# groupeLIAMG/ttcr

Measured on AMD Instinct MI355X. Metric: Mnodes/s per sweep-iteration (512^3 fp32 grid, first-order FSM), higher is better.
Workload: dtype f32

## Files before the change

ttcr_amd/csrc/fsm_capi.hip:

```cpp
#include <hip/hip_runtime.h>

#include <algorithm>
#include <atomic>
#include <chrono>
#include <condition_variable>
#include <cmath>
#include <cstdio>
#include <cstdlib>
#include <cstring>
#include <limits>
#include <map>
#include <memory>
#include <mutex>
#include <sstream>
#include <stdexcept>
#include <string>
#include <thread>
#include <vector>

#include "../../include/ttcr_amd.h"
#include "fsm_kernels.h"
#include "fsm_fast_api.h"
#include "fsm_tape_api.h"
#include "fsm_adjoint_api.h"
// ... 492 lines not shown
                    const int ja = std::max(j0 - 2 * H, 0), jb = std::min(jm + 2 * H, geom.NJ - 1);
                    const int ka = std::max(k0 - 2 * H, 0), kb = std::min(km + 2 * H, geom.NK - 1);
                    const int ja2 = rj != prj ? geom.NJ - 1 - jb : ja, jb2 = rj != prj ? geom.NJ - 1 - ja : jb;
                    const int ka2 = rk != prk ? geom.NK - 1 - kb : ka, kb2 = rk != prk ? geom.NK - 1 - ka : kb;
                    for (int tk = ka2 / PK; tk <= kb2 / PK; ++tk)
                        for (int tj = ja2 / PJ; tj <= jb2 / PJ; ++tj) t = std::max(t, tf[(size_t)(d - 1) * n_patches + (size_t)tk * npj + tj]);
                }
                ts[me] = t;
                tf[me] = t + ((jm - j0) + (km - k0) + geom.NF + C - 1) / C + 1.0;
            }
        }
        std::vector<uint32_t> idx((size_t)n_patches * ndir);
        size_t q = 0;
        std::vector<uint32_t> ent((size_t)n_patches * ndir);
        std::vector<double> key((size_t)n_patches * ndir);
        for (int d = 0; d < ndir; ++d)
            for (uint32_t e : diag_order) {
                const int TJ = e & 0xffffu, TK = e >> 16;
                ent[q] = (uint32_t)TJ | ((uint32_t)TK << 14) | ((uint32_t)d << 28);
                key[q] = ts[(size_t)d * n_patches + (size_t)TK * npj + TJ];
                idx[q] = (uint32_t)q;
                ++q;
            }
        std::stable_sort(idx.begin(), idx.end(), [&](uint32_t a2, uint32_t b2) { return key[a2] < key[b2]; });
        for (uint32_t i2 : idx) out.push_back(ent[i2]);
        return out;
    }

    template <int DIM, int H>
    void launch_sweeps_persistent(int batch) {
        constexpr int C0 = ChunkCfg<T, DIM>::C;
        if constexpr (DIM == 3 && C0 == 8) {
            const int below = H == 2 ? weno_c16_below : sizeof(T) == 4 ? std::numeric_limits<int>::max() : f64_c16_below;
            if (NS == 1 && mode == 2 && (lone_chunk == 16 || fast_now<H>()) && batch < below) {
                launch_sweeps_persistent_ns<DIM, H, 1, 16, true>(batch);
                return;
            }
        }
        if (H == 2 && DIM == 3 && NS == 2 && batch >= weno_ch4_min && C0 == 8) {
            if (NS == 2) launch_sweeps_persistent_ns<DIM, H, 2, (H == 2 && DIM == 3) ? 4 : C0>(batch);
            else launch_sweeps_persistent_ns<DIM, H, 1, (H == 2 && DIM == 3) ? 4 : C0>(batch);
        } else {
            if (NS == 2) launch_sweeps_persistent_ns<DIM, H, 2, C0>(batch); else launch_sweeps_persistent_ns<DIM, H, 1, C0>(batch);
        }
    }

    template <int DIM, int H, int NSV, int CH, bool XS_ONLY = false>
    void launch_sweeps_persistent_ns(int batch) {
        using C = TileCfg<T, DIM>;
        PersistArgs<T> pa;
        SweepArgs<T>& a = pa.s;
        constexpr bool NO_PRE = CH == 16 && H == 1 && DIM == 3;
        const size_t dyn_lds = NO_PRE ? 0 : xs_dyn_lds(batch);
        a.tt = d_tt.p;
        a.ts = NS;
        a.lmask = d_lmask.p;
        a.frozen = d_mask.p;
        a.bbox = d_bbox.p;
        a.change = d_change.p;
        a.slots = d_slots.p;
        a.tiles = nullptr;
        a.g = geom;
        a.prof = d_prof.p;
        a.mask_words = (uint32_t)mask_words;
        a.dx = dx;
        a.dz = dz;
        a.w = 0;
        a.variant = DIM == 3 ? 0 : (dx == dz ? 1 : 2);
        pa.order = d_order.p;
        pa.sync = d_sync.p;
        pa.n_patches = n_patches;
        pa.batch = batch;
        pa.timeout_ticks = 300000000ull;
        pa.stamp = d_stamp.p;
        pa.iter_ptr = d_iter.p;
        pa.evals = d_evals.p;
        pa.nbf = nbf; pa.nbj = nbj; pa.nbk = nbk;
        pa.ndir = DIM == 3 ? 8 : 4;
        pa.skip = skip_now(batch) ? (std::getenv("TTCR_FSM_SKIP_ALL_DIRTY") ? 2 : 1) : 0;
        pa.cmap = d_cmap.p;
        pa.cw = cmap_words;
        pa.sw = std::getenv("TTCR_FSM_NO_SW") ? nullptr : d_sw.p;
        pa.n_sw_groups = n_groups();
        pa.n_sw_sweeps = sw_sweeps;

        const size_t wg_cap = (fsm_looped(DIM == 3, H) && persist_wgs > 0) ? (size_t)persist_wgs : ~(size_t)0;
        const dim3 block(C::PJ * C::PK), grid((unsigned)std::min<size_t>((size_t)n_patches * batch, wg_cap));
        const int ndir = DIM == 3 ? 8 : 4;
        {
            const bool pre_ = mode == 2 && !NO_PRE && (DIM == 2 || batch >= pre_min || dyn_lds > 0);
            char nm[160];
            std::snprintf(nm, sizeof nm, "fsm_sweep_persistent<%s,%d,%d,%d,%s,%s,%d,%d,%s,%s>", sizeof(T) == 4 ? "float" : "double", C::PJ, C::PK, CH,
                          DIM == 3 ? "true" : "false", skip_now(batch) ? "true" : "false", H, NSV, mode == 2 ? "true" : "false", pre_ ? "true" : "false");
            last_kernel = nm;
        }
        if (mode == 2) {
            pa.ssh = d_ssh.p;
            pa.ssh_stride = ssh_stride;
            pa.dir = 0;
            a.rf = a.rj = a.rk = a.rev = 0;
            a.s_sheared = nullptr;
            pa.timeout_ticks = 1000000000ull;
            const dim3 gridx((unsigned)std::min<size_t>((size_t)n_patches * batch * ndir, wg_cap));
            pa.order = d_order_xs[H == 2 ? 1 : 0][batch < time_order_below ? 1 : 0].p;
            const bool pre = DIM == 2 || batch >= pre_min || dyn_lds > 0;
            if constexpr (std::is_same<T, float>::value) {
                if (fast_now<H>() && (H == 1 || NSV == 1)) {
                    const FastCfg fc{H, DIM, NSV, CH, skip_now(batch), NO_PRE ? false : pre};
                    last_kernel.insert(last_kernel.size() - 1, ",1");
                    const hipError_t e = fsm_fast_launch(pa, fc, gridx.x, dyn_lds, stream);
                    if (e == hipErrorInvalidValue) throw std::logic_error("arith = 1: no such kernel (" + last_kernel + ")");
                    HIP_CHECK(e);
                    return;
                }
            }
            if constexpr (NO_PRE) {
                (void)pre;
                if (skip_now(batch))
                    fsm_sweep_persistent<T, C::PJ, C::PK, CH, DIM == 3, true, H, NSV, true><<<gridx, block, dyn_lds, stream>>>(pa);
                else
                    fsm_sweep_persistent<T, C::PJ, C::PK, CH, DIM == 3, false, H, NSV, true><<<gridx, block, dyn_lds, stream>>>(pa);
            } else {
                if (skip_now(batch) && pre)
                    fsm_sweep_persistent<T, C::PJ, C::PK, CH, DIM == 3, true, H, NSV, true, true><<<gridx, block, dyn_lds, stream>>>(pa);
                else if (skip_now(batch))
                    fsm_sweep_persistent<T, C::PJ, C::PK, CH, DIM == 3, true, H, NSV, true><<<gridx, block, dyn_lds, stream>>>(pa);
                else if (pre)
                    fsm_sweep_persistent<T, C::PJ, C::PK, CH, DIM == 3, false, H, NSV, true, true><<<gridx, block, dyn_lds, stream>>>(pa);
                else
                    fsm_sweep_persistent<T, C::PJ, C::PK, CH, DIM == 3, false, H, NSV, true><<<gridx, block, dyn_lds, stream>>>(pa);
            }
            HIP_CHECK(hipGetLastError());
            return;
        }
        if (fast_now<H>() && H == 1) throw ValueError("option 'arith' = 1 needs whole-iteration launches (option 'mode' = 2)");
        if constexpr (XS_ONLY) throw std::logic_error("launch_sweeps_persistent_ns: whole-iteration launches only");
        else {
        pa.ssh = nullptr;
        pa.ssh_stride = 0;
        static const int RX2[4] = {0, 1, 1, 0}, RZ2[4] = {0, 0, 1, 1};
        for (int d = 0; d < ndir; ++d) {
            int fam;
            if (DIM == 3) {
                a.rf = d & 1; a.rj = (d >> 1) & 1; a.rk = (d >> 2) & 1;
                a.rev = a.rk;
                fam = (a.rf ^ a.rk) | ((a.rj ^ a.rk) << 1);
            } else {
                a.rj = RX2[d]; a.rf = RZ2[d]; a.rk = 0;
                a.rev = a.rj;
                fam = a.rf ^ a.rj;
            }
            a.s_sheared = d_ssh.p + (size_t)fam * ssh_stride;
            pa.dir = d;
            if (skip_now(batch))
                fsm_sweep_persistent<T, C::PJ, C::PK, CH, DIM == 3, true, H, NSV, false><<<grid, block, 0, stream>>>(pa);
            else
                fsm_sweep_persistent<T, C::PJ, C::PK, CH, DIM == 3, false, H, NSV, false><<<grid, block, 0, stream>>>(pa);
        }
        HIP_CHECK(hipGetLastError());
        }
    }

    void build_tile_lists(int PJ, int PK, int BL) {
        std::vector<uint32_t> all;
        tile_off.assign(n_launch, 0);
        tile_cnt.assign(n_launch, 0);
        for (int w = 0; w < n_launch; ++w) {
            tile_off[w] = (int)all.size();
            for (int m = 0; m <= geom.npj + geom.npk - 2; ++m) {
                const int L0 = BL * w - m * (BL - 1);
                for (int TK = std::max(0, m - geom.npj + 1); TK <= std::min(m, geom.npk - 1); ++TK) {
                    const int TJ = m - TK;
                    const int j0 = TJ * PJ, k0 = TK * PK;
                    const int jmaxp = std::min(j0 + PJ, geom.NJ) - 1, kmaxp = std::min(k0 + PK, geom.NK) - 1;
// ... 3350 lines not shown
```

ttcr_amd/csrc/fsm_fast.hip:

```cpp
#include "fsm_fast_api.h"

namespace ttcr_amd {

template <int PJ, int PK, int C, bool IS3D, bool SKIP, int NS, bool PRE, int H = 1>
static hipError_t launch_one(const PersistArgs<float>& pa, unsigned wgs, size_t dyn_lds, hipStream_t stream) {
    fsm_sweep_persistent<float, PJ, PK, C, IS3D, SKIP, H, NS, true, PRE, 1><<<dim3(wgs), dim3(PJ * PK), dyn_lds, stream>>>(pa);
    return hipGetLastError();
}

hipError_t fsm_fast_launch(const PersistArgs<float>& pa, const FastCfg& c, unsigned wgs, size_t dyn_lds, hipStream_t stream) {
    if (c.h == 2) {
#ifndef FSM_FAST_MIN
        if (c.ns != 1) return hipErrorInvalidValue;
        if (c.dim == 3 && c.chunk == 16) {
            if (c.skip) return c.pre ? launch_one<16, 16, 16, true, true, 1, true, 2>(pa, wgs, dyn_lds, stream)
                                     : launch_one<16, 16, 16, true, true, 1, false, 2>(pa, wgs, dyn_lds, stream);
            return c.pre ? launch_one<16, 16, 16, true, false, 1, true, 2>(pa, wgs, dyn_lds, stream)
                         : launch_one<16, 16, 16, true, false, 1, false, 2>(pa, wgs, dyn_lds, stream);
        }
        if (c.dim == 3 && c.chunk == 8) {
            if (c.skip) return c.pre ? launch_one<16, 16, 8, true, true, 1, true, 2>(pa, wgs, dyn_lds, stream)
                                     : launch_one<16, 16, 8, true, true, 1, false, 2>(pa, wgs, dyn_lds, stream);
            return c.pre ? launch_one<16, 16, 8, true, false, 1, true, 2>(pa, wgs, dyn_lds, stream)
                         : launch_one<16, 16, 8, true, false, 1, false, 2>(pa, wgs, dyn_lds, stream);
        }
        if (c.dim == 2 && c.chunk == 16 && c.pre)
            return c.skip ? launch_one<64, 1, 16, false, true, 1, true, 2>(pa, wgs, dyn_lds, stream)
                          : launch_one<64, 1, 16, false, false, 1, true, 2>(pa, wgs, dyn_lds, stream);
#endif
        return hipErrorInvalidValue;
    }
    if (c.dim == 3 && c.ns == 1 && c.chunk == 16 && !c.pre)
        return c.skip ? launch_one<16, 16, 16, true, true, 1, false>(pa, wgs, dyn_lds, stream)
                      : launch_one<16, 16, 16, true, false, 1, false>(pa, wgs, dyn_lds, stream);
#ifndef FSM_FAST_MIN
    if (c.dim == 3 && c.ns == 2 && c.chunk == 8) {
        if (c.skip) return c.pre ? launch_one<16, 16, 8, true, true, 2, true>(pa, wgs, dyn_lds, stream)
                                 : launch_one<16, 16, 8, true, true, 2, false>(pa, wgs, dyn_lds, stream);
        return c.pre ? launch_one<16, 16, 8, true, false, 2, true>(pa, wgs, dyn_lds, stream)
                     : launch_one<16, 16, 8, true, false, 2, false>(pa, wgs, dyn_lds, stream);
    }
    if (c.dim == 2 && c.ns == 1 && c.chunk == 16 && c.pre)
        return c.skip ? launch_one<64, 1, 16, false, true, 1, true>(pa, wgs, dyn_lds, stream)
                      : launch_one<64, 1, 16, false, false, 1, true>(pa, wgs, dyn_lds, stream);
#endif
    return hipErrorInvalidValue;
}

}
```

ttcr_amd/csrc/fsm_fast_api.h:

```cpp
#pragma once
#include "fsm_kernels.h"

namespace ttcr_amd {

struct FastCfg {
    int h;
    int dim;
    int ns;
    int chunk;
    bool skip;
    bool pre;
};
hipError_t fsm_fast_launch(const PersistArgs<float>& pa, const FastCfg& c, unsigned wgs, size_t dyn_lds, hipStream_t stream);

}
```

ttcr_amd/csrc/fsm_kernels.h:

```cpp
#pragma once
#include <hip/hip_runtime.h>
#include <stdint.h>
#include <type_traits>

namespace ttcr_amd {

constexpr int FSM_BRICK = 16;

template <typename T> struct real_traits;
template <> struct real_traits<float> {
    static __host__ __device__ constexpr float max() { return 3.402823466e+38f; }
    static __device__ __forceinline__ float inf() { return __builtin_huge_valf(); }
};
template <> struct real_traits<double> {
    static __host__ __device__ constexpr double max() { return 1.7976931348623157e+308; }
    static __device__ __forceinline__ double inf() { return __builtin_huge_val(); }
};

__device__ __forceinline__ uint32_t idx_u32(double v) { return v < 0 ? 0u : (v >= 4294967295.0 ? 4294967295u : (uint32_t)v); }

__device__ __forceinline__ float rmin(float a, float b) { return a < b ? a : b; }
__device__ __forceinline__ double rmin(double a, double b) { return a < b ? a : b; }
__device__ __forceinline__ float rmax(float a, float b) { return a < b ? b : a; }
__device__ __forceinline__ double rmax(double a, double b) { return a < b ? b : a; }
// ... 691 lines not shown
__device__ __forceinline__ float lane_above(float x, float edge) {
    return __uint_as_float((unsigned)__builtin_amdgcn_update_dpp((int)__float_as_uint(edge), (int)__float_as_uint(x), 0x130, 0xf, 0xf, false));
}
__device__ __forceinline__ double lane_below(double x, double edge) {
    const unsigned long long u = (unsigned long long)__double_as_longlong(x), e = (unsigned long long)__double_as_longlong(edge);
    const unsigned lo = (unsigned)__builtin_amdgcn_update_dpp((int)(unsigned)e, (int)(unsigned)u, 0x138, 0xf, 0xf, false);
    const unsigned hi = (unsigned)__builtin_amdgcn_update_dpp((int)(unsigned)(e >> 32), (int)(unsigned)(u >> 32), 0x138, 0xf, 0xf, false);
    return __longlong_as_double((long long)(((unsigned long long)hi << 32) | lo));
}
__device__ __forceinline__ double lane_above(double x, double edge) {
    const unsigned long long u = (unsigned long long)__double_as_longlong(x), e = (unsigned long long)__double_as_longlong(edge);
    const unsigned lo = (unsigned)__builtin_amdgcn_update_dpp((int)(unsigned)e, (int)(unsigned)u, 0x130, 0xf, 0xf, false);
    const unsigned hi = (unsigned)__builtin_amdgcn_update_dpp((int)(unsigned)(e >> 32), (int)(unsigned)(u >> 32), 0x130, 0xf, 0xf, false);
    return __longlong_as_double((long long)(((unsigned long long)hi << 32) | lo));
}

template <typename T, int NS> struct Pack;
template <typename T> struct Pack<T, 1> { T v[1]; };
template <typename T> struct alignas(2 * sizeof(T)) Pack<T, 2> { T v[2]; };

template <typename T, int NS>
__device__ __forceinline__ Pack<T, NS> pack_fill(T x) {
    Pack<T, NS> p;
#pragma unroll
    for (int l = 0; l < NS; ++l) p.v[l] = x;
    return p;
}
__device__ __forceinline__ Pack<float, 1> ld_sc1(const Pack<float, 1>* p) { Pack<float, 1> r; r.v[0] = ld_sc1(&p->v[0]); return r; }
__device__ __forceinline__ Pack<double, 1> ld_sc1(const Pack<double, 1>* p) { Pack<double, 1> r; r.v[0] = ld_sc1(&p->v[0]); return r; }
__device__ __forceinline__ Pack<float, 2> ld_sc1(const Pack<float, 2>* p) {
    const unsigned long long u = __hip_atomic_load((const unsigned long long*)p, __ATOMIC_RELAXED, __HIP_MEMORY_SCOPE_AGENT);
    Pack<float, 2> r;
    r.v[0] = __uint_as_float((unsigned)u);
    r.v[1] = __uint_as_float((unsigned)(u >> 32));
    return r;
}
__device__ __forceinline__ Pack<double, 2> ld_sc1(const Pack<double, 2>* p) {
    Pack<double, 2> r;
    r.v[0] = ld_sc1(&p->v[0]);
    r.v[1] = ld_sc1(&p->v[1]);
    return r;
}
__device__ __forceinline__ void st_sc1(Pack<float, 1>* p, Pack<float, 1> x) { st_sc1(&p->v[0], x.v[0]); }
__device__ __forceinline__ void st_sc1(Pack<double, 1>* p, Pack<double, 1> x) { st_sc1(&p->v[0], x.v[0]); }
__device__ __forceinline__ void st_sc1(Pack<float, 2>* p, Pack<float, 2> x) {
    const unsigned long long u = (unsigned long long)__float_as_uint(x.v[0]) | ((unsigned long long)__float_as_uint(x.v[1]) << 32);
    __hip_atomic_store((unsigned long long*)p, u, __ATOMIC_RELAXED, __HIP_MEMORY_SCOPE_AGENT);
}
__device__ __forceinline__ void st_sc1(Pack<double, 2>* p, Pack<double, 2> x) {
    st_sc1(&p->v[0], x.v[0]);
    st_sc1(&p->v[1], x.v[1]);
}

__host__ __device__ constexpr bool fsm_looped(bool is3d, int h) { return is3d && h == 1; }

__device__ __forceinline__ int kmaxp_of(int k0, int NK, int PK) { return (k0 + PK < NK ? k0 + PK : NK) - 1; }
template <typename T, int PJ, int PK, int C, bool IS3D, bool SKIP, int H, int NS, bool XS, bool PRE, int AR = 0>
__device__ __forceinline__ bool fsm_sweep_unit(const PersistArgs<T>& pa) {
    static_assert(AR == 0 || std::is_same<T, float>::value, "tolerance-grade arithmetic: fp32 kernels");
    constexpr bool LOOPED = fsm_looped(IS3D, H);
    using P = Pack<T, NS>;
    constexpr int NT = PJ * PK;
    constexpr int RJ = PJ + 2 * H;
    constexpr int NROWS = IS3D ? RJ * (PK + 2 * H) : RJ;
    constexpr int NQ = C + 2 * H;
    constexpr int RS = NQ | 1;
    constexpr int NUP = IS3D ? H * (PJ + PK) : H;
    constexpr int NDH = IS3D ? H * (PJ + PK) : H;
    constexpr int RPI = NT / C;
    constexpr int NOWN = C;
    constexpr int NHI = (NDH + RPI - 1) / RPI;
    constexpr int NUPI = (NUP + RPI - 1) / RPI;
    static_assert(NT % C == 0 && (IS3D || PK == 1) && C <= FSM_BRICK && (H == 1 || H == 2), "tile shape");
    static_assert(C - 1 <= FSM_XPAD, "the rows of a chunk are read from the sheared copies without a wrap");
    static_assert(!(SKIP && FSM_EARLY_PUB > 0), "FSM_EARLY_PUB is a tuning option of the kernels without exact skipping");
    const SweepArgs<T>& a = pa.s;
    const unsigned epoch = (unsigned)pa.iter_ptr[1] + (XS ? 0u : (unsigned)pa.dir);
    const int e2 = (int)(epoch % 3u) + 1;
    auto dec_prog = [&](int raw_) -> int { return (int)((unsigned)raw_ >> 30) == e2 ? (raw_ & 0x3fffffff) : 0; };
    auto ld_raw = [&](const int* p_) -> int { return __hip_atomic_load(p_, __ATOMIC_RELAXED, __HIP_MEMORY_SCOPE_AGENT); };
    auto ld_prog = [&](const int* p_) -> int { return dec_prog(ld_raw(p_)); };
    auto st_prog = [&](int* p_, int v_) {
        __hip_atomic_store(p_, (int)(((unsigned)e2 << 30) | (unsigned)v_), __ATOMIC_RELAXED, __HIP_MEMORY_SCOPE_AGENT);
    };
    auto ld_cmap = [&](const unsigned long long* p_) -> unsigned {
        const unsigned long long v_ = __hip_atomic_load(p_, __ATOMIC_RELAXED, __HIP_MEMORY_SCOPE_AGENT);
        return (unsigned)(v_ >> 32) == epoch ? (unsigned)v_ : 0u;
    };
    auto st_cmap = [&](unsigned long long* p_, unsigned v_) {
        __hip_atomic_store(p_, ((unsigned long long)epoch << 32) | v_, __ATOMIC_RELAXED, __HIP_MEMORY_SCOPE_AGENT);
    };

    __shared__ P Tt[NROWS * RS];
    __shared__ int s_ticket, s_abort;
    __shared__ int s_anychg;
    constexpr int SLABW = SKIP ? FSM_SLAB_WORDS : 1;
    __shared__ unsigned s_stamped[SKIP ? 9 : 1][SLABW];
    __shared__ unsigned s_slab[SLABW];
    __shared__ int s_next, s_act;
    __shared__ int s_cwi[2], s_cwl[2];
    __shared__ unsigned s_cwv[2];
    __shared__ int s_mywi;
    __shared__ unsigned s_mywv[2];
    enum { U_THR, U_RSJLO, U_RSKLO, U_RSNJ, U_RSNK, U_LCF, U_UPLCF0, U_UPLCF1, U_HIST, U_EVER, U_UCHG, U_PENDV, U_LCHG, U_N };
    __shared__ int s_u[U_N];

    int tid = threadIdx.x;
    if constexpr (LOOPED) asm volatile("" : "+v"(tid));
    unsigned long long prof_t = (FSM_ENABLE_PROF && a.prof) ? wall_clock64() : 0ull;
    unsigned long long pacc[6] = {0, 0, 0, 0, 0, 0};
    unsigned pchunks = 0;
    unsigned long long twait = 0;
// ... 217 lines not shown
        abase[it] = nat_row(jq, kq) + (uint32_t)(rf ? NF - 1 - b : b);
        lrow[it] = lds_row(cj, ck) + e + 2 * H;
    }
    int uipb[NUPI];
    uint32_t uabase[NUPI];
    int ulrow[NUPI];
#pragma unroll
    for (int it = 0; it < NUPI; ++it) {
        const int h = rsub + RPI * it;
        int cj, ck;
        bool ok = h < NUP;
        if (IS3D) {
            if (h < H * PK) { cj = -1 - h / PK; ck = h % PK; } else { cj = (h - H * PK) % PJ; ck = -1 - (h - H * PK) / PJ; }
        } else {
            cj = -1 - h; ck = 0;
        }
        const int jq = j0 + cj, kq = k0 + ck;
        ok = ok && jq >= 0 && jq < NJ && kq >= 0 && kq < NK;
        const int b = -1 + e - jq - kq;
        uipb[it] = ok ? b : -(1 << 29);
        uabase[it] = nat_row(jq >= 0 ? jq : 0, kq >= 0 ? kq : 0) + (uint32_t)(rf ? NF - 1 - b : b);
        ulrow[it] = (h < NUP) ? lds_row(cj, ck) + e + H - 1 : -1;
    }
    int xipb = -(1 << 29), xlrow = -1;
    uint32_t xabase = 0;
    bool x_up = false;
    if (H == 2) {
        constexpr int NX1 = IS3D ? (PJ + PK) : 1;
        static_assert(H != 2 || 3 * NX1 <= NT, "extras fit one pass");
        if (tid < 3 * NX1) {
            const bool up = tid >= NX1;
            const int dist = tid >= 2 * NX1 ? 2 : 1;
            const int h = tid % NX1;
            int cj, ck;
            if (IS3D) {
                if (h < PK) { cj = up ? -dist : PJ; ck = h; } else { cj = h - PK; ck = up ? -dist : PK; }
            } else {
                cj = up ? -dist : PJ; ck = 0;
            }
            const int jq = j0 + cj, kq = k0 + ck;
            const bool ok = jq >= 0 && jq < NJ && kq >= 0 && kq < NK;
            const int lev = up ? -2 : 1;
            const int b = lev - jq - kq;
            xipb = ok ? b : -(1 << 29);
            xabase = nat_row(jq >= 0 ? jq : 0, kq >= 0 ? kq : 0) + (uint32_t)(rf ? NF - 1 - b : b);
            xlrow = lds_row(cj, ck) + lev + H;
            x_up = up;
        }
    }

    const int m = TJ + TK;
    int Lc = Ls - (((Ls - m) % C + C) % C);

    T sv[C];
    P tv[NOWN + NHI];
    int xs_next = 0, xs_level = -(1 << 30);
    auto issue_static = [&](int L) {
        int x;
        if (L == xs_level) {
            x = xs_next;
        } else {
            x = (rev ? NF + NJ + NK - 3 - L : L) % M;
            x = x < 0 ? x + M : x;
        }
        x = __builtin_amdgcn_readfirstlane(x);
        int xlo = rev ? x - (C - 1) : x;
        if (xlo < 0) { xlo %= M; xlo = xlo < 0 ? xlo + M : xlo; }
        constexpr bool paired = IS3D;
        const uint32_t SRB = (paired ? (uint32_t)a.g.SR : (uint32_t)NJ) * (uint32_t)sizeof(T);
        const char* rowp = reinterpret_cast<const char*>(Sg + (size_t)skx_min * shear_plane(a.g)) + (size_t)(paired ? (uint32_t)xlo >> 1 : (uint32_t)xlo) * SRB;
        auto ld_row = [&](int half) -> T {
            asm volatile("" : "+s"(rowp));
            return *reinterpret_cast<const T*>(rowp + half * 16 * (int)sizeof(T) + stoff);
        };
        if constexpr (paired) {
            if ((xlo & 1) == 0) {
#pragma unroll
                for (int q = 0; q < C; ++q) {
                    sv[q] = ld_row(q & 1);
                    if (q & 1) rowp += SRB;
                }
            } else {
#pragma unroll
                for (int q = 0; q < C; ++q) {
                    if (!(q & 1)) { sv[q] = ld_row(1); rowp += SRB; } else sv[q] = ld_row(0);
                }
            }
        } else {
#pragma unroll
            for (int q = 0; q < C; ++q) {
                sv[q] = ld_row(0);
                rowp += SRB;
            }
        }
        x = rev ? x - C : x + C;
        if (x < 0 || x >= M) { x %= M; x = x < 0 ? x + M : x; }
        xs_next = x;
        xs_level = L + C;
        const int sL = sf * L;
#pragma unroll
        for (int it = 0; it < NOWN + NHI; ++it) {
            P v = PFILL;
            if ((unsigned)(L + ipb[it]) < (unsigned)NF) v = XS ? ld_sc1(Tg + (abase[it] + sL)) : Tg[abase[it] + sL];
            tv[it] = v;
        }
    };

    unsigned long long nevals = 0;

    T dec[NS];
#pragma unroll
    for (int l = 0; l < NS; ++l) dec[l] = 0;
    P carry[2 * H];
#pragma unroll
    for (int q = 0; q < 2 * H; ++q) carry[q] = PFILL;
    bool have_prev = false;
    int pref_for = -(1 << 30);
    int pending = 0;
    int n_done = 0;
    int pre_j = -1, pre_k = -1;
    int smp_j = 0, smp_k = 0;
    P uvn[NUPI];
    int uvn_for = -(1 << 30);
    int near_lo[NS], near_hi[NS];
    {
        const int jlo = rj ? NJ - 1 - jmaxp : j0, jhi = rj ? NJ - 1 - j0 : jmaxp;
        const int klo = rk ? NK - 1 - kmaxp : k0, khi = rk ? NK - 1 - k0 : kmaxp;
#pragma unroll
        for (int l = 0; l < NS; ++l) {
            const int* b6 = bb + 6 * l;
            const int b0 = rf ? NF - 1 - b6[1] : b6[0], b1 = rf ? NF - 1 - b6[0] : b6[1];
            const bool jk = !(jhi < b6[2] || jlo > b6[3] || khi < b6[4] || klo > b6[5]) && b0 <= NF - 1 && b1 >= 0;
            near_lo[l] = jk ? b0 - (C - 1) + j0 + k0 : 1;
            near_hi[l] = jk ? b1 + jmaxp + kmaxp : 0;
        }
    }
    if (!FSM_EXP_NOWAIT && XS && dir > 0 && !chase) {
        if (tid < 16) {
            const int* pp = prev_sweep_counter(dir, TJ, TK, z, tid);
            if (pp) {
                const unsigned long long t0 = wall_clock64();
                int spins = 0;
                while (ld_prog(pp) < (SKIP ? FSM_FIN : 0x3fffffff)) {
                    if ((++spins & 63) == 0) {
                        if (__hip_atomic_load(pa.sync + 4, __ATOMIC_RELAXED, __HIP_MEMORY_SCOPE_AGENT)) break;
                        if (wall_clock64() - t0 > pa.timeout_ticks) {
                            __hip_atomic_store(pa.sync + 4, 1, __ATOMIC_RELAXED, __HIP_MEMORY_SCOPE_AGENT);
                            break;
                        }
                    }
                    __builtin_amdgcn_s_sleep(8);
                }
            }
        }
        __syncthreads();
    }
    if (CHASE_OK && chase) chase_wait(Lc - C, -1, false);
    if (!SKIP) { issue_static(Lc); pref_for = Lc; }
    if constexpr (SKIP) {
        const int nsw = (pa.nbf + 31) >> 5;
        for (int w = tid; w < nsw; w += NT) s_slab[w] = 0u;
        for (int w = tid; w < 9 * SLABW; w += NT) s_stamped[w / SLABW][w % SLABW] = 0u;
        if (tid == 0) {
            s_cwi[0] = -1; s_cwi[1] = -1; s_mywi = -1;
            const int ja = j0 - H < 0 ? 0 : j0 - H, jb = jmaxp + H > NJ - 1 ? NJ - 1 : jmaxp + H;
            const int ka = k0 - H < 0 ? 0 : k0 - H, kb = kmaxp + H > NK - 1 ? NK - 1 : kmaxp + H;
            const int jlo = (rj ? NJ - 1 - jb : ja) / FSM_BRICK, jhi = (rj ? NJ - 1 - ja : jb) / FSM_BRICK;
            const int klo = (rk ? NK - 1 - kb : ka) / FSM_BRICK, khi = (rk ? NK - 1 - ka : kb) / FSM_BRICK;
            s_u[U_RSJLO] = jlo; s_u[U_RSNJ] = jhi - jlo + 1;
            s_u[U_RSKLO] = klo; s_u[U_RSNK] = khi - klo + 1;
            const int sg = pa.ndir * pa.iter_ptr[0] + dir + 1;
            s_u[U_THR] = pa.skip == 2 ? -(1 << 30) : (sg - 1 > 0 ? sg - 1 : 0);
            s_u[U_LCF] = Lc;
            const int lsj = Ls - PJ, lsk = Ls - PK, mu = TJ + TK - 1;
// ... 142 lines not shown
            }
            __syncthreads();
            const int act = __builtin_amdgcn_readfirstlane(s_act), Ln = __builtin_amdgcn_readfirstlane(s_next);
            if (Ln != Lc) {
                have_prev = false;
                Lc = Ln;
            }
            if (act == 2) {
                asm volatile("s_waitcnt vmcnt(0)" ::: "memory");
                __syncthreads();
                if (tid == 0) st_prog(my_prog, s_u[U_PENDV]);
                pending = 0;
                Lc -= C;
                continue;
            }
            if (act == 0) break;
        }
        const int L0 = Lc;
        const int eoff = jp + kp - L0;
        const int ea = col_ok ? (eoff > 0 ? eoff : 0) : C;
        const int eb = eoff + NF - 1 < C - 1 ? eoff + NF - 1 : C - 1;
        if constexpr (!SKIP) { FSM_PMARK(0) }

        if constexpr (!SKIP) {
        if (CHASE_OK && chase) {
            chase_wait(L0, pre_j, true);
        } else if (tid == 0 && (up_j || up_k) && !((up_j ? pre_j : 0x3fffffff) >= L0 + C - 1 && (up_k ? pre_k : 0x3fffffff) >= L0 + C - 1)) {
            const int need = L0 + C - 1;
            unsigned long long t0 = 0;
            int spins = 0;
            for (;;) {
                const int vj = up_j ? ld_prog(up_j) : need;
                const int vk = up_k ? ld_prog(up_k) : need;
                if (vj >= need && vk >= need) break;
                if (spins == 0) t0 = wall_clock64();
                if ((++spins & 63) == 0) {
                    if (__hip_atomic_load(pa.sync + 4, __ATOMIC_RELAXED, __HIP_MEMORY_SCOPE_AGENT)) break;
                    if (wall_clock64() - t0 > pa.timeout_ticks) {
                        __hip_atomic_store(pa.sync + 4, 1, __ATOMIC_RELAXED, __HIP_MEMORY_SCOPE_AGENT);
                        break;
                    }
                }
                __builtin_amdgcn_s_sleep(FSM_POLL_SLEEP);
            }
        }
        __syncthreads();
        }
        if (tid == 0) s_anychg = 0;
        FSM_PMARK(1)
        if (pref_for != L0) issue_static(L0);
        nevals += (eb >= ea) ? (unsigned)(eb - ea + 1) : 0u;

        P uv[NUPI];
        if (PRE && uvn_for == L0) {
#pragma unroll
            for (int it = 0; it < NUPI; ++it) uv[it] = uvn[it];
        } else {
#pragma unroll
            for (int it = 0; it < NUPI; ++it) {
                P v = PFILL;
                if ((unsigned)(L0 + uipb[it]) < (unsigned)NF) v = ld_sc1(Tg + (uabase[it] + sf * L0));
                uv[it] = v;
            }
        }
        P xv = PFILL;
        if (H == 2 && (unsigned)(L0 + xipb) < (unsigned)NF) {
            const P* src = Tg + (xabase + sf * L0);
            if (x_up || XS) xv = ld_sc1(src); else xv = *src;
        }
#pragma unroll
        for (int it = 0; it < NOWN + NHI; ++it)
            if (it < NOWN || rsub + RPI * (it - NOWN) < NDH) Tt[lrow[it]] = tv[it];
        if (!have_prev) {
#pragma unroll
            for (int q = 0; q < 2 * H; ++q) {
                const int ip = L0 - H + q - jp - kp;
                P v = PFILL;
                if (col_ok && (unsigned)ip < (unsigned)NF) {
                    const P* src = Tg + (colbase + (rf ? NF - 1 - ip : ip));
                    v = XS ? ld_sc1(src) : *src;
                }
                carry[q] = v;
            }
            have_prev = true;
        }
#pragma unroll
        for (int q = 0; q < 2 * H; ++q) Tt[row * RS + q] = carry[q];
        asm volatile("s_waitcnt vmcnt(0)" ::: "memory");
#pragma unroll
        for (int it = 0; it < NUPI; ++it)
            if (ulrow[it] >= 0) Tt[ulrow[it]] = uv[it];
        if (H == 2 && xlrow >= 0) Tt[xlrow] = xv;
        __syncthreads();
        if (tid == 0 && pending) st_prog(my_prog, SKIP ? s_u[U_PENDV] : pending);
        pending = 0;
        if (PRE && Lc + C <= Le) {
            const int need_n = SKIP ? (L0 + 2 * C - 1) << 8 : L0 + 2 * C - 1;
            const int sj = up_j ? __builtin_amdgcn_readfirstlane(pre_j) : 0x7fffffff;
            const int sk = up_k ? __builtin_amdgcn_readfirstlane(pre_k) : 0x7fffffff;
            if (sj >= need_n && sk >= need_n) {
#pragma unroll
                for (int it = 0; it < NUPI; ++it) {
                    P v = PFILL;
                    if ((unsigned)(L0 + C + uipb[it]) < (unsigned)NF) v = ld_sc1(Tg + (uabase[it] + sf * (L0 + C)));
                    uvn[it] = v;
                }
                uvn_for = L0 + C;
            }
        }
        if (PRE && (tid & 63) == 0 && Lc + C <= Le) {
            if (up_j) smp_j = ld_raw(up_j);
            if (up_k) smp_k = ld_raw(up_k);
        }
        if (PRE && CHASE_OK && chase_ptr && Lc + C <= Le)
            smp_j = ld_raw(chase_ptr);

        bool near_src[NS];
#pragma unroll
        for (int l = 0; l < NS; ++l) near_src[l] = L0 >= near_lo[l] && L0 <= near_hi[l];

        P own[NQ];
#pragma unroll
        for (int q = 0; q < 2 * H; ++q) own[q] = carry[q];
#pragma unroll
        for (int q = 2 * H; q < NQ; ++q) own[q] = Tt[row * RS + q];
        T sc[C];
#pragma unroll
        for (int q = 0; q < C; ++q) sc[q] = rev ? sv[C - 1 - q] : sv[q];
        FSM_PMARK(2)

        if (Lc + C <= Le) { issue_static(Lc + C); pref_for = Lc + C; }

        constexpr bool WAVE2D = !IS3D && NT == 64 && H == 1;
        P hup[WAVE2D ? C : 1], hdn[WAVE2D ? C : 1];
        if (WAVE2D) {
#pragma unroll
            for (int ee = 0; ee < C; ++ee) {
                hup[ee] = Tt[(H - 1) * RS + ee + H - 1];
                hdn[ee] = Tt[(PJ + H) * RS + ee + H + 1];
            }
        }
        bool changed = false;
        constexpr bool DUP = H == 1 && !IS3D;
        if constexpr (!DUP) {
#define FSM_SIMPLE false
#define FSM_VAR 0
#include "fsm_march_levels.inc"
#undef FSM_SIMPLE
#undef FSM_VAR
        } else {
            bool near_any = false;
#pragma unroll
            for (int l = 0; l < NS; ++l) near_any |= near_src[l];
            const bool full_wave = !near_any && __builtin_amdgcn_ballot_w64(ea == 0 && eb == C - 1) == ~0ull;
            if (!full_wave) {
#define FSM_SIMPLE false
#define FSM_VAR 0
#include "fsm_march_levels.inc"
#undef FSM_SIMPLE
#undef FSM_VAR
            } else if (variant == 1) {
#define FSM_SIMPLE true
#define FSM_VAR 1
#include "fsm_march_levels.inc"
#undef FSM_SIMPLE
#undef FSM_VAR
            } else {
#define FSM_SIMPLE true
#define FSM_VAR 2
#include "fsm_march_levels.inc"
#undef FSM_SIMPLE
#undef FSM_VAR
            }
        }
#pragma unroll
        for (int q = 0; q < 2 * H; ++q) carry[q] = own[C + q];
        FSM_PMARK(3)
        if (FSM_ENABLE_PROF) ++pchunks;

        if constexpr (SKIP) {
            const bool ej = changed && jp + H > jmaxp, ek = IS3D && changed && kp + H > kmaxp;
            const int f = (wave_any(changed) ? 1 : 0) | (wave_any(ej) ? 2 : 0) | (wave_any(ek) ? 4 : 0);
            if (f && (tid & 63) == 0) atomicOr(&s_anychg, f);
            if (!(FSM_SKIP_ABL & 2) && changed) {
                const int ip0 = L0 - jp - kp;
                const int ia = ip0 + ea, ib = ip0 + eb;
                const int ba = (rf ? NF - 1 - ib : ia) / FSM_BRICK, bb2 = (rf ? NF - 1 - ia : ib) / FSM_BRICK;
                const int my_bj = (rj ? NJ - 1 - jp : jp) / FSM_BRICK - s_u[U_RSJLO], my_bk = (rk ? NK - 1 - kp : kp) / FSM_BRICK - s_u[U_RSKLO];
                const int jk = my_bk * s_u[U_RSNJ] + my_bj;
                atomicOr(&s_stamped[jk][ba >> 5], 1u << (ba & 31));
                if (bb2 != ba) atomicOr(&s_stamped[jk][bb2 >> 5], 1u << (bb2 & 31));
            }
        } else {
            if (wave_any(changed) && (tid & 63) == 0) s_anychg = 1;
        }
        __syncthreads();
        const int chg_flags = SKIP ? __builtin_amdgcn_readfirstlane(s_anychg) : s_anychg;
        const bool any_changed = chg_flags != 0;
        if (any_changed) {
#pragma unroll
            for (int it = 0; it < NOWN; ++it) {
                const int ipm = L0 + ipb[it] - H;
                if ((unsigned)ipm < (unsigned)NF) {
                    const int rid = rsub + RPI * it;
                    const int cj = rid % PJ, ck = rid / PJ;
                    P* dst = Tg + (abase[it] + sf * (L0 - H));
                    const P v = Tt[lrow[it] - H];
                    if (XS || cj >= PJ - H || (IS3D && ck >= PK - H)) st_sc1(dst, v); else *dst = v;
                }
            }
        }
        if constexpr (SKIP) {
            if (!(FSM_SKIP_ABL & 4) && tid == 0) {
                if (any_changed) {
                    int flo, fhi;
                    chunk_frange(L0, 0, flo, fhi);
                    for (int b = flo / FSM_BRICK; b <= fhi / FSM_BRICK; ++b) s_slab[b >> 5] |= 1u << (b & 31);
                    const int ci = (L0 - s_u[U_LCF]) / C, w = ci >> 5;
                    if ((chg_flags & 6) && w < pa.cw) {
                        if (s_mywi != w) { s_mywi = w; s_mywv[0] = 0u; s_mywv[1] = 0u; }
                        for (int e2 = 0; e2 < 2; ++e2)
                            if (chg_flags & (2 << e2)) {
                                s_mywv[e2] |= 1u << (ci & 31);
                                st_cmap(cmap_of(TK * npj + TJ, e2) + w, s_mywv[e2]);
                            }
                    }
                    s_u[U_UCHG] = 1;
                    s_u[U_LCHG] = 1;
                }
                const int h2 = ((s_u[U_HIST] << 2) | (chg_flags >> 1)) & 0xff, ev2 = s_u[U_EVER] | (chg_flags >> 1);
                s_u[U_HIST] = h2;
                s_u[U_EVER] = ev2;
                s_u[U_PENDV] = Lc + C > Le ? (FSM_FIN | ev2) : (((Lc + C) << 8) | h2);
            }
        }
        if constexpr (SKIP) pending = 1;
        else pending = Lc + C > Le ? 0x3fffffff : Lc + C;
        if (FSM_EARLY_PUB > 0 && n_done < FSM_EARLY_PUB) {
            asm volatile("s_waitcnt vmcnt(0)" ::: "memory");
            __syncthreads();
            if (tid == 0) st_prog(my_prog, SKIP ? s_u[U_PENDV] : pending);
            pending = 0;
        }
        ++n_done;
        FSM_PMARK(4)
    }
    if constexpr (SKIP) {
        __syncthreads();
        if (s_u[U_UCHG]) {
            const int nsw = (pa.nbf + 31) >> 5;
            const int rs_jlo = s_u[U_RSJLO], rs_nj = s_u[U_RSNJ], rs_klo = s_u[U_RSKLO], njk = rs_nj * s_u[U_RSNK];
            int* __restrict__ stamp = pa.stamp + (size_t)grp * pa.nbf * pa.nbj * pa.nbk;
// ... 15 lines not shown
        const int sigma0 = pa.ndir * pa.iter_ptr[0] + dir;
        if (tid == 0 && pa.sw && sigma0 < pa.n_sw_sweeps)
            atomicAdd(pa.sw + (size_t)sigma0 * pa.n_sw_groups + grp, 1ull | (s_u[U_UCHG] ? (1ull << 32) : 0ull));
    }

    if (FSM_ENABLE_PROF && a.prof && tid == 0) {
        if constexpr (FSM_ENABLE_PROF == 2) {
            for (int q = 0; q < 6; ++q) atomicAdd(a.prof + q, s_pacc[q]);
            atomicAdd(a.prof + 6, 1ull);
            atomicAdd(a.prof + 7, (unsigned long long)pchunks);
        }
        if (FSM_ENABLE_PROF == 1) {
#pragma unroll
            for (int q = 0; q < 6; ++q) atomicAdd(a.prof + q, pacc[q]);
            atomicAdd(a.prof + 6, 1ull);
            atomicAdd(a.prof + 7, (unsigned long long)pchunks);
        }
        if (ticket < FSM_TRACE_UNITS) {
            unsigned long long* tr = a.prof + 8 + 4 * (size_t)ticket;
            tr[0] = trace_t0; tr[1] = FSM_ENABLE_PROF == 2 ? ((trace_t1 - trace_t0) & 0xffffffffull) | (twait << 32) : trace_t1; tr[2] = wall_clock64();
            tr[3] = (unsigned long long)TJ | ((unsigned long long)TK << 16) | ((unsigned long long)dir << 32) | ((unsigned long long)z << 40) |
                    ((unsigned long long)pchunks << 48);
        }
    }
#undef FSM_PMARK
#pragma unroll
    for (int off = 32; off > 0; off >>= 1) nevals += __shfl_down(nevals, off, 64);
#pragma unroll
    for (int l = 0; l < NS; ++l) {
        double accd = (double)dec[l];
#pragma unroll
        for (int off = 32; off > 0; off >>= 1) accd += __shfl_down(accd, off, 64);
        if ((tid & 63) == 0 && accd != 0.0) atomicAdd(a.change + grp * NS + l, accd);
        if ((tid & 63) == 0 && nevals && ((lm >> l) & 1)) atomicAdd(pa.evals + grp * NS + l, nevals);
    }
    return true;
}

template <typename T, int PJ, int PK, int C, bool IS3D, bool SKIP, int H, int NS, bool XS, bool PRE = false, int AR = 0>
#ifndef FSM_WENO_MINW
#define FSM_WENO_MINW FSM_MINW
#endif
__global__ __launch_bounds__(PJ* PK, (SKIP && IS3D && H == 1 && NS == 2 && sizeof(T) == 4) ? 3
                                     : (IS3D && H == 2 && NS == 1 && sizeof(T) == 4) ? FSM_WENO_MINW : FSM_MINW) void fsm_sweep_persistent(const PersistArgs<T> pa) {
    if constexpr (fsm_looped(IS3D, H)) {
        (void)pa;
        for (;;) {
            auto kp = __builtin_amdgcn_kernarg_segment_ptr();
            asm volatile("" : "+s"(kp));
            if (!fsm_sweep_unit<T, PJ, PK, C, IS3D, SKIP, H, NS, XS, PRE, AR>(*(const PersistArgs<T>*)kp)) break;
        }
    } else {
        fsm_sweep_unit<T, PJ, PK, C, IS3D, SKIP, H, NS, XS, PRE, AR>(pa);
    }
}

template <typename T>
struct Sweep45Args {
    T* tt;
    const T* s;
    const uint32_t* frozen;
    double* change;
    const int* slots;
    const int* lmask;
    int ts, by_group;
    int nnx, nnz;
    size_t n_nodes;
    uint32_t mask_words;
    T dx;
};

template <typename T, int NT>
__global__ __launch_bounds__(NT) void fsm_sweep45(const Sweep45Args<T> a) {
    constexpr int W = 16, C = 8;
    __shared__ T ring[NT * W];
    int slot;
    if (a.by_group) {
        const int z = blockIdx.x / a.ts, l = blockIdx.x % a.ts;
        const int grp = a.slots[z];
        if (grp < 0 || !((a.lmask[z] >> l) & 1)) return;
        slot = grp * a.ts + l;
    } else {
        slot = a.slots[blockIdx.x];
        if (slot < 0) return;
    }
    T* __restrict__ Tg = a.tt + ((size_t)(slot / a.ts) * a.n_nodes * a.ts + slot % a.ts);
    const uint32_t* __restrict__ Fz = a.frozen + (size_t)slot * a.mask_words;
    const int nnx = a.nnx, nnz = a.nnz, ts = a.ts;
    const T TMAX = real_traits<T>::max();
    const int r = threadIdx.x;
    constexpr int S = NT - 2;
    T dec = 0;
    for (int dir = 0; dir < 4; ++dir) {
        const int ri = (dir == 1) | (dir == 2), rj = dir >> 1;
        for (int x0 = 0; x0 < nnx; x0 += S) {
            const int ncol = nnx - x0 < S ? nnx - x0 : S;
            const int nlev = 2 * (ncol - 1) + nnz;
            const int xp = x0 + r - 1;
            const bool col_in = xp >= 0 && xp < nnx && r <= ncol + 1;
            const bool own = r >= 1 && r <= ncol;
            const int i = ri ? nnx - 1 - xp : xp;
            const uint32_t rowbase = (uint32_t)(col_in ? i : 0) * nnz;
            auto load_levels = [&](int lo, T* v) {
#pragma unroll
                for (int e = 0; e < C; ++e) {
                    const int zp = lo + e - 2 * (r - 1);
// ... 1724 lines not shown
```

Measured before the change: 93910.

## Add wide 16-byte buffer-load/store streaming path for fp32 two-source FSM sweeps

Adds a WIDE variant of the persistent sweep kernel for fp32, 3-D, first-order, two-source, chunk-8 configurations. Each lane loads and stores two adjacent nodes (two float pairs) with 128-bit raw buffer loads and stores instead of per-node 8-byte accesses, using a remapped thread-to-column layout for the tile, halo and upwind rows. The goal is fewer, wider memory transactions in the bandwidth-bound sweep. The cost is complex index remapping, odd-alignment special cases, and conditions on even NF, 16-byte alignment and a field size under 4 GiB.

```diff
diff --git a/ttcr_amd/csrc/fsm_capi.hip b/ttcr_amd/csrc/fsm_capi.hip
--- a/ttcr_amd/csrc/fsm_capi.hip
+++ b/ttcr_amd/csrc/fsm_capi.hip
@@ -568,6 +568,10 @@
         SweepArgs<T>& a = pa.s;
         constexpr bool NO_PRE = CH == 16 && H == 1 && DIM == 3;
         const size_t dyn_lds = NO_PRE ? 0 : xs_dyn_lds(batch);
+        constexpr bool WIDE_OK = std::is_same<T, float>::value && DIM == 3 && H == 1 && NSV == 2 && CH == 8;
+        const bool wide = WIDE_OK && mode == 2 && geom.NF % 2 == 0 && ((uintptr_t)d_tt.p & 15u) == 0 &&
+                          (unsigned long long)geom.n_nodes * 2ull * sizeof(T) < (1ull << 32) &&
+                          !std::getenv("TTCR_FSM_NARROW");
         a.tt = d_tt.p;
         a.ts = NS;
         a.lmask = d_lmask.p;
@@ -606,7 +610,7 @@
         {
             const bool pre_ = mode == 2 && !NO_PRE && (DIM == 2 || batch >= pre_min || dyn_lds > 0);
             char nm[160];
-            std::snprintf(nm, sizeof nm, "fsm_sweep_persistent<%s,%d,%d,%d,%s,%s,%d,%d,%s,%s>", sizeof(T) == 4 ? "float" : "double", C::PJ, C::PK, CH,
+            std::snprintf(nm, sizeof nm, "fsm_sweep_persistent%s<%s,%d,%d,%d,%s,%s,%d,%d,%s,%s>", wide ? "_wide" : "", sizeof(T) == 4 ? "float" : "double", C::PJ, C::PK, CH,
                           DIM == 3 ? "true" : "false", skip_now(batch) ? "true" : "false", H, NSV, mode == 2 ? "true" : "false", pre_ ? "true" : "false");
             last_kernel = nm;
         }
@@ -622,7 +626,7 @@
             const bool pre = DIM == 2 || batch >= pre_min || dyn_lds > 0;
             if constexpr (std::is_same<T, float>::value) {
                 if (fast_now<H>() && (H == 1 || NSV == 1)) {
-                    const FastCfg fc{H, DIM, NSV, CH, skip_now(batch), NO_PRE ? false : pre};
+                    const FastCfg fc{H, DIM, NSV, CH, skip_now(batch), NO_PRE ? false : pre, wide};
                     last_kernel.insert(last_kernel.size() - 1, ",1");
                     const hipError_t e = fsm_fast_launch(pa, fc, gridx.x, dyn_lds, stream);
                     if (e == hipErrorInvalidValue) throw std::logic_error("arith = 1: no such kernel (" + last_kernel + ")");
@@ -636,6 +640,17 @@
                     fsm_sweep_persistent<T, C::PJ, C::PK, CH, DIM == 3, true, H, NSV, true><<<gridx, block, dyn_lds, stream>>>(pa);
                 else
                     fsm_sweep_persistent<T, C::PJ, C::PK, CH, DIM == 3, false, H, NSV, true><<<gridx, block, dyn_lds, stream>>>(pa);
+            } else if (wide) {
+                if constexpr (WIDE_OK) {
+                    if (skip_now(batch) && pre)
+                        fsm_sweep_persistent_wide<T, C::PJ, C::PK, CH, DIM == 3, true, H, NSV, true, true><<<gridx, block, dyn_lds, stream>>>(pa);
+                    else if (skip_now(batch))
+                        fsm_sweep_persistent_wide<T, C::PJ, C::PK, CH, DIM == 3, true, H, NSV, true><<<gridx, block, dyn_lds, stream>>>(pa);
+                    else if (pre)
+                        fsm_sweep_persistent_wide<T, C::PJ, C::PK, CH, DIM == 3, false, H, NSV, true, true><<<gridx, block, dyn_lds, stream>>>(pa);
+                    else
+                        fsm_sweep_persistent_wide<T, C::PJ, C::PK, CH, DIM == 3, false, H, NSV, true><<<gridx, block, dyn_lds, stream>>>(pa);
+                }
             } else {
                 if (skip_now(batch) && pre)
                     fsm_sweep_persistent<T, C::PJ, C::PK, CH, DIM == 3, true, H, NSV, true, true><<<gridx, block, dyn_lds, stream>>>(pa);
diff --git a/ttcr_amd/csrc/fsm_fast.hip b/ttcr_amd/csrc/fsm_fast.hip
--- a/ttcr_amd/csrc/fsm_fast.hip
+++ b/ttcr_amd/csrc/fsm_fast.hip
@@ -8,7 +8,14 @@
     return hipGetLastError();
 }
 
+template <bool SKIP, bool PRE>
+static hipError_t launch_wide(const PersistArgs<float>& pa, unsigned wgs, size_t dyn_lds, hipStream_t stream) {
+    fsm_sweep_persistent_wide<float, 16, 16, 8, true, SKIP, 1, 2, true, PRE, 1><<<dim3(wgs), dim3(256), dyn_lds, stream>>>(pa);
+    return hipGetLastError();
+}
+
 hipError_t fsm_fast_launch(const PersistArgs<float>& pa, const FastCfg& c, unsigned wgs, size_t dyn_lds, hipStream_t stream) {
+    if (c.wide && !(c.h == 1 && c.dim == 3 && c.ns == 2 && c.chunk == 8)) return hipErrorInvalidValue;
     if (c.h == 2) {
 #ifndef FSM_FAST_MIN
         if (c.ns != 1) return hipErrorInvalidValue;
@@ -35,6 +42,10 @@
                       : launch_one<16, 16, 16, true, false, 1, false>(pa, wgs, dyn_lds, stream);
 #ifndef FSM_FAST_MIN
     if (c.dim == 3 && c.ns == 2 && c.chunk == 8) {
+        if (c.wide) {
+            if (c.skip) return c.pre ? launch_wide<true, true>(pa, wgs, dyn_lds, stream) : launch_wide<true, false>(pa, wgs, dyn_lds, stream);
+            return c.pre ? launch_wide<false, true>(pa, wgs, dyn_lds, stream) : launch_wide<false, false>(pa, wgs, dyn_lds, stream);
+        }
         if (c.skip) return c.pre ? launch_one<16, 16, 8, true, true, 2, true>(pa, wgs, dyn_lds, stream)
                                  : launch_one<16, 16, 8, true, true, 2, false>(pa, wgs, dyn_lds, stream);
         return c.pre ? launch_one<16, 16, 8, true, false, 2, true>(pa, wgs, dyn_lds, stream)
diff --git a/ttcr_amd/csrc/fsm_fast_api.h b/ttcr_amd/csrc/fsm_fast_api.h
--- a/ttcr_amd/csrc/fsm_fast_api.h
+++ b/ttcr_amd/csrc/fsm_fast_api.h
@@ -10,6 +10,7 @@
     int chunk;
     bool skip;
     bool pre;
+    bool wide;
 };
 hipError_t fsm_fast_launch(const PersistArgs<float>& pa, const FastCfg& c, unsigned wgs, size_t dyn_lds, hipStream_t stream);
 
diff --git a/ttcr_amd/csrc/fsm_kernels.h b/ttcr_amd/csrc/fsm_kernels.h
--- a/ttcr_amd/csrc/fsm_kernels.h
+++ b/ttcr_amd/csrc/fsm_kernels.h
@@ -767,12 +767,39 @@
     st_sc1(&p->v[1], x.v[1]);
 }
 
+typedef unsigned int fsm_u32x4 __attribute__((ext_vector_type(4)));
+__device__ __forceinline__ __amdgpu_buffer_rsrc_t pair_field_rsrc(Pack<float, 2>* tg, uint32_t n_nodes) {
+    return __builtin_amdgcn_make_buffer_rsrc((void*)tg, 0, (int)(n_nodes * (uint32_t)sizeof(Pack<float, 2>)), 0x00020000);
+}
+__device__ __forceinline__ fsm_u32x4 ld16_sc1(__amdgpu_buffer_rsrc_t r, uint32_t node) {
+    return __builtin_amdgcn_raw_buffer_load_b128(r, (int)(node * (uint32_t)sizeof(Pack<float, 2>)), 0, 16);
+}
+__device__ __forceinline__ void st16_sc1(__amdgpu_buffer_rsrc_t r, uint32_t node, Pack<float, 2> lo, Pack<float, 2> hi) {
+    fsm_u32x4 v;
+    v.x = __float_as_uint(lo.v[0]); v.y = __float_as_uint(lo.v[1]); v.z = __float_as_uint(hi.v[0]); v.w = __float_as_uint(hi.v[1]);
+    __builtin_amdgcn_raw_buffer_store_b128(v, r, (int)(node * (uint32_t)sizeof(Pack<float, 2>)), 0, 16);
+}
+__device__ __forceinline__ void st8_sc1(__amdgpu_buffer_rsrc_t r, uint32_t node, Pack<float, 2> x) {
+    typedef unsigned int u32x2 __attribute__((ext_vector_type(2)));
+    u32x2 v;
+    v.x = __float_as_uint(x.v[0]); v.y = __float_as_uint(x.v[1]);
+    __builtin_amdgcn_raw_buffer_store_b64(v, r, (int)(node * (uint32_t)sizeof(Pack<float, 2>)), 0, 16);
+}
+__device__ __forceinline__ Pack<float, 2> pair_half(fsm_u32x4 v, int half) {
+    Pack<float, 2> r;
+    r.v[0] = __uint_as_float(half ? v.z : v.x);
+    r.v[1] = __uint_as_float(half ? v.w : v.y);
+    return r;
+}
+
 __host__ __device__ constexpr bool fsm_looped(bool is3d, int h) { return is3d && h == 1; }
 
 __device__ __forceinline__ int kmaxp_of(int k0, int NK, int PK) { return (k0 + PK < NK ? k0 + PK : NK) - 1; }
-template <typename T, int PJ, int PK, int C, bool IS3D, bool SKIP, int H, int NS, bool XS, bool PRE, int AR = 0>
+template <typename T, int PJ, int PK, int C, bool IS3D, bool SKIP, int H, int NS, bool XS, bool PRE, int AR = 0, bool WIDE = false>
 __device__ __forceinline__ bool fsm_sweep_unit(const PersistArgs<T>& pa) {
     static_assert(AR == 0 || std::is_same<T, float>::value, "tolerance-grade arithmetic: fp32 kernels");
+    static_assert(!WIDE || (std::is_same<T, float>::value && NS == 2 && H == 1 && IS3D && C == 8 && PJ == 16 && PK == 16 && XS),
+                  "wide streaming map: fp32 source pairs, first order, 3-D, chunks of 8 levels, whole-iteration launches");
     constexpr bool LOOPED = fsm_looped(IS3D, H);
     using P = Pack<T, NS>;
     constexpr int NT = PJ * PK;
@@ -1096,8 +1123,70 @@
     const int m = TJ + TK;
     int Lc = Ls - (((Ls - m) % C + C) % C);
 
+    constexpr int NWI = WIDE ? 3 : 1;
+    int wn[NWI];
+    uint32_t wab[NWI];
+    int wlr[NWI];
+    unsigned wok = 0;
+    bool wodd = false;
+    const int wkq = k0 + (tid >> 6);
+    const int wdab = (rk ? -4 : 4) * NJ * NF - 4 * sf;
+    auto w_slot = [](int it) { return it < 4 ? 0 : it - 3; };
+    auto w_n = [&](int it) { return it < 4 ? ((wkq + 4 * it < NK) ? wn[0] - 4 * sf * it : -(1 << 29)) : wn[it - 3]; };
+    auto w_ab = [&](int it) { return it < 4 ? wab[0] + (uint32_t)(it * wdab) : wab[it - 3]; };
+    auto w_lr = [&](int it) {
+        int b = wlr[w_slot(it)];
+        asm volatile("" : "+v"(b));
+        return it < 4 ? b + it * 4 * RJ * RS : b;
+    };
+    if constexpr (WIDE) {
+        static_assert(!WIDE || (NT == 256 && NUP == 32 && NDH == 32), "wide streaming map: 16 x 16 columns");
+        auto wide_item = [&](int it, int cj, int ck, int loff, int k, bool slot) -> bool {
+            const int jq = j0 + cj, kq = k0 + ck;
+            const bool ok = slot && jq >= 0 && jq < NJ && kq >= 0 && kq < NK;
+            const int ip0 = Lc + loff - jq - kq;
+            const int w0 = rf ? NF - C - ip0 : ip0;
+            const int n = (w0 & ~1) + 2 * k;
+            const int ql = (rf ? NF - 1 - n : n) + jq + kq - Lc + H;
+            const int qa = loff > 0 ? 2 * H : 0, qb = qa + C - 1;
+            const bool lo = slot && ql >= qa && ql <= qb, hi = slot && ql + sf >= qa && ql + sf <= qb;
+            wn[it] = (ok && (lo || hi)) ? n - sf * Lc : -(1 << 29);
+            wab[it] = nat_row(jq, kq) + (uint32_t)(n - sf * Lc);
+            wlr[it] = lds_row(cj, ck) + ql;
+            wok |= ((lo ? 1u : 0u) | (hi ? 2u : 0u)) << (2 * it);
+            return (w0 & 1) != 0;
+        };
+        static_assert(!WIDE || PJ * 4 == 64, "passes 0..3: the lane's column keeps its j', k' moves by 4");
+        auto dn_col = [&](int h, int& cj, int& ck) { if (h < PK) { cj = PJ; ck = h; } else { cj = h - PK; ck = PK; } };
+        wodd = wide_item(0, (tid >> 2) % PJ, (tid >> 2) / PJ, H, tid & 3, true);
+        if (tid < 128) {
+            const int ck = tid >> 3;
+            wide_item(1, 2 * (tid & 7) + ((Lc - ck) & 1), ck, H, 4, true);
+        } else {
+            int cj, ck;
+            dn_col((tid - 128) >> 2, cj, ck);
+            wide_item(1, cj, ck, H, tid & 3, true);
+        }
+        if (tid < 160) {
+            const int h = tid & 31;
+            wide_item(2, h < PK ? -1 : h - PK, h < PK ? h : -1, -1, tid >> 5, true);
+        } else {
+            int cj, ck;
+            dn_col((tid - 160) & 31, cj, ck);
+            wide_item(2, cj, ck, H, 4, tid < 192);
+        }
+    }
+
     T sv[C];
-    P tv[NOWN + NHI];
+    P tv[WIDE ? 1 : NOWN + NHI];
+    fsm_u32x4 tw[WIDE ? 5 : 1];
+    const fsm_u32x4 WINF = {0x7f800000u, 0x7f800000u, 0x7f800000u, 0x7f800000u};
+    auto wide_put = [&](int it, fsm_u32x4 v) {
+        if constexpr (WIDE) {
+            if (wok & (1u << (2 * w_slot(it)))) Tt[w_lr(it)] = pair_half(v, 0);
+            if (wok & (2u << (2 * w_slot(it)))) Tt[w_lr(it) + sf] = pair_half(v, 1);
+        }
+    };
     int xs_next = 0, xs_level = -(1 << 30);
     auto issue_static = [&](int L) {
         int x;
@@ -1142,11 +1231,21 @@
         xs_next = x;
         xs_level = L + C;
         const int sL = sf * L;
+        if constexpr (WIDE) {
+            const __amdgpu_buffer_rsrc_t trs = pair_field_rsrc(Tg, (uint32_t)a.g.n_nodes);
+#pragma unroll
+            for (int it = 0; it < 5; ++it) {
+                fsm_u32x4 v = WINF;
+                if ((unsigned)(w_n(it) + sL) < (unsigned)NF) v = ld16_sc1(trs, w_ab(it) + (uint32_t)sL);
+                tw[it] = v;
+            }
+        } else {
 #pragma unroll
         for (int it = 0; it < NOWN + NHI; ++it) {
             P v = PFILL;
             if ((unsigned)(L + ipb[it]) < (unsigned)NF) v = XS ? ld_sc1(Tg + (abase[it] + sL)) : Tg[abase[it] + sL];
             tv[it] = v;
+        }
         }
     };
 
@@ -1164,6 +1263,7 @@
     int n_done = 0;
     int pre_j = -1, pre_k = -1;
     int smp_j = 0, smp_k = 0;
+    fsm_u32x4 uwn = WINF;
     P uvn[NUPI];
     int uvn_for = -(1 << 30);
     int near_lo[NS], near_hi[NS];
@@ -1412,6 +1512,14 @@
         nevals += (eb >= ea) ? (unsigned)(eb - ea + 1) : 0u;
 
         P uv[NUPI];
+        fsm_u32x4 uw = WINF;
+        if constexpr (WIDE) {
+            if (PRE && uvn_for == L0) {
+                uw = uwn;
+            } else if ((unsigned)(w_n(5) + sf * L0) < (unsigned)NF) {
+                uw = ld16_sc1(pair_field_rsrc(Tg, (uint32_t)a.g.n_nodes), w_ab(5) + (uint32_t)(sf * L0));
+            }
+        } else {
         if (PRE && uvn_for == L0) {
 #pragma unroll
             for (int it = 0; it < NUPI; ++it) uv[it] = uvn[it];
@@ -1423,14 +1531,20 @@
                 uv[it] = v;
             }
         }
+        }
         P xv = PFILL;
         if (H == 2 && (unsigned)(L0 + xipb) < (unsigned)NF) {
             const P* src = Tg + (xabase + sf * L0);
             if (x_up || XS) xv = ld_sc1(src); else xv = *src;
         }
+        if constexpr (WIDE) {
+#pragma unroll
+            for (int it = 0; it < 5; ++it) wide_put(it, tw[it]);
+        } else {
 #pragma unroll
         for (int it = 0; it < NOWN + NHI; ++it)
             if (it < NOWN || rsub + RPI * (it - NOWN) < NDH) Tt[lrow[it]] = tv[it];
+        }
         if (!have_prev) {
 #pragma unroll
             for (int q = 0; q < 2 * H; ++q) {
@@ -1447,9 +1561,13 @@
 #pragma unroll
         for (int q = 0; q < 2 * H; ++q) Tt[row * RS + q] = carry[q];
         asm volatile("s_waitcnt vmcnt(0)" ::: "memory");
+        if constexpr (WIDE) {
+            wide_put(5, uw);
+        } else {
 #pragma unroll
         for (int it = 0; it < NUPI; ++it)
             if (ulrow[it] >= 0) Tt[ulrow[it]] = uv[it];
+        }
         if (H == 2 && xlrow >= 0) Tt[xlrow] = xv;
         __syncthreads();
         if (tid == 0 && pending) st_prog(my_prog, SKIP ? s_u[U_PENDV] : pending);
@@ -1459,11 +1577,17 @@
             const int sj = up_j ? __builtin_amdgcn_readfirstlane(pre_j) : 0x7fffffff;
             const int sk = up_k ? __builtin_amdgcn_readfirstlane(pre_k) : 0x7fffffff;
             if (sj >= need_n && sk >= need_n) {
+                if constexpr (WIDE) {
+                    uwn = WINF;
+                    if ((unsigned)(w_n(5) + sf * (L0 + C)) < (unsigned)NF)
+                        uwn = ld16_sc1(pair_field_rsrc(Tg, (uint32_t)a.g.n_nodes), w_ab(5) + (uint32_t)(sf * (L0 + C)));
+                } else {
 #pragma unroll
                 for (int it = 0; it < NUPI; ++it) {
                     P v = PFILL;
                     if ((unsigned)(L0 + C + uipb[it]) < (unsigned)NF) v = ld_sc1(Tg + (uabase[it] + sf * (L0 + C)));
                     uvn[it] = v;
+                }
                 }
                 uvn_for = L0 + C;
             }
@@ -1557,7 +1681,24 @@
         __syncthreads();
         const int chg_flags = SKIP ? __builtin_amdgcn_readfirstlane(s_anychg) : s_anychg;
         const bool any_changed = chg_flags != 0;
-        if (any_changed) {
+        if (WIDE && any_changed) {
+            if constexpr (WIDE) {
+                const __amdgpu_buffer_rsrc_t trs = pair_field_rsrc(Tg, (uint32_t)a.g.n_nodes);
+                const int sh = sf * L0 + (rf ? 2 : 0);
+#pragma unroll
+                for (int it = 0; it < 4; ++it) {
+                    const int n = w_n(it) + sh;
+                    const uint32_t ad = w_ab(it) + (uint32_t)sh;
+                    const int lr = w_lr(it) - (rf ? 2 : 0);
+                    if (wodd || (tid & 3) != 3) {
+                        if ((unsigned)n < (unsigned)NF) st16_sc1(trs, ad, Tt[lr], Tt[lr + sf]);
+                    } else {
+                        if ((unsigned)n < (unsigned)NF) st8_sc1(trs, ad, Tt[lr]);
+                        if ((unsigned)(n - 7) < (unsigned)NF) st8_sc1(trs, ad - 7u, Tt[lr - 7 * sf]);
+                    }
+                }
+            }
+        } else if (any_changed) {
 #pragma unroll
             for (int it = 0; it < NOWN; ++it) {
                 const int ipm = L0 + ipb[it] - H;
@@ -1679,6 +1820,16 @@
         }
     } else {
         fsm_sweep_unit<T, PJ, PK, C, IS3D, SKIP, H, NS, XS, PRE, AR>(pa);
+    }
+}
+
+template <typename T, int PJ, int PK, int C, bool IS3D, bool SKIP, int H, int NS, bool XS, bool PRE = false, int AR = 0>
+__global__ __launch_bounds__(PJ* PK, SKIP ? 3 : FSM_MINW) void fsm_sweep_persistent_wide(const PersistArgs<T> pa) {
+    (void)pa;
+    for (;;) {
+        auto kp = __builtin_amdgcn_kernarg_segment_ptr();
+        asm volatile("" : "+s"(kp));
+        if (!fsm_sweep_unit<T, PJ, PK, C, IS3D, SKIP, H, NS, XS, PRE, AR, true>(*(const PersistArgs<T>*)kp)) break;
     }
 }
 
```

Result: slower. 80700 (-14.1%).
